# BloodAxe/segmentation-networks-benchmark

Measured on AMD Instinct MI355X. Metric: images/sec/GPU (fwd+bwd) ZF_UNET 224x224 bs=32; 1/2/4/8-GPU scaling, higher is better.
Workload: dtype bf16; 1 GPU; ZF_UNET 224x224 bf16 bs=32/GPU, bce_dice, SGD lr 1e-3, Dropout2d 0.2, train step torch_train.py:180-190 (configs[1]); global_batch=32, parallelism=dp1

## Files before the change

segmentation-networks-benchmark_amd/csrc/common.h:

```cpp
#pragma once
#include <hip/hip_runtime.h>
#include <hip/hip_ext.h>
#include <limits.h>
#include <stdint.h>
#include <stdio.h>
#include <string.h>

#include "../../include/segnb_hip.h"

typedef __attribute__((ext_vector_type(8))) __bf16 bf16x8_t;
typedef __attribute__((ext_vector_type(16))) float f32x16_t;

struct bf16_t {
    unsigned short bits;
};

void segnb_set_error(const char* fmt, ...);

#define SEGNB_CHECK_ARG_AS(who, cond, msg)                           \
    do {                                                             \
        if (!(cond)) {                                               \
            segnb_set_error("%s: bad argument: %s", who, msg);       \
            return SEGNB_E_BADARG;                                   \
        }                                                            \
// ... 35 lines not shown
inline T segnb_plan_keep(T v) {
    static_assert(!(std::is_pointer<T>::value && std::is_class<typename std::remove_pointer<T>::type>::value),
                  "segnb_plan_keep: add an overload that copies this struct into the plan");
    return v;
}
inline const segnb_conv_geom* segnb_plan_keep(const segnb_conv_geom* g) {
    return g ? (const segnb_conv_geom*)segnb_plan_dup(g, sizeof(*g)) : g;
}
inline const segnb_loss_spec* segnb_plan_keep(const segnb_loss_spec* g) {
    return g ? (const segnb_loss_spec*)segnb_plan_dup(g, sizeof(*g)) : g;
}
inline const segnb_bn_reduce_epilogue* segnb_plan_keep(const segnb_bn_reduce_epilogue* g) {
    return g ? (const segnb_bn_reduce_epilogue*)segnb_plan_dup(g, sizeof(*g)) : g;
}
inline const segnb_bn_apply_epilogue* segnb_plan_keep(const segnb_bn_apply_epilogue* g) {
    return g ? (const segnb_bn_apply_epilogue*)segnb_plan_dup(g, sizeof(*g)) : g;
}
inline const segnb_upcat_src* segnb_plan_keep(const segnb_upcat_src* g) {
    return g ? (const segnb_upcat_src*)segnb_plan_dup(g, sizeof(*g)) : g;
}
inline const segnb_operand_tf* segnb_plan_keep(const segnb_operand_tf* g) {
    return g ? (const segnb_operand_tf*)segnb_plan_dup(g, sizeof(*g)) : g;
}
inline const segnb_wgrad_target* segnb_plan_keep(const segnb_wgrad_target* g) {
    return g ? (const segnb_wgrad_target*)segnb_plan_dup(g, sizeof(*g)) : g;
}
inline const segnb_act_epilogue* segnb_plan_keep(const segnb_act_epilogue* g) {
    return g ? (const segnb_act_epilogue*)segnb_plan_dup(g, sizeof(*g)) : g;
}
template <class... P, class... A>
inline void segnb_plan_record_call(const char* name, int (*fn)(P...), A... args) {
    static_assert(sizeof...(P) == sizeof...(A), "argument count");
    std::tuple<P...> kept(segnb_plan_keep((P)args)...);
    segnb_plan_push([fn, kept]() { return std::apply(fn, kept); }, name);
}
extern int g_segnb_census_on;
void segnb_census(const char* name);
#define SEGNB_PLAN_RECORD(fn, ...)                                                           \
    SegnbPlanScope plan_scope__;                                                             \
    if (plan_scope__.top && g_segnb_census_on) segnb_census(#fn);                            \
    if (plan_scope__.top && segnb_plan_recording()) segnb_plan_record_call(#fn, fn, __VA_ARGS__)
void segnb_plan_refuse(const char* why);
#define SEGNB_PLAN_REFUSE(why)                                         \
    SegnbPlanScope plan_scope__;                                       \
    if (plan_scope__.top && g_segnb_census_on) segnb_census(__func__); \
    if (plan_scope__.top && segnb_plan_recording()) segnb_plan_refuse(why)

int segnb_num_cus();
bool segnb_fprop_general_forced();
int segnb_knob_fprop_dma();
int segnb_knob_fprop_dma_cfg();
int segnb_knob_fprop_dma_dbg();
int segnb_knob_fprop_dma_epi();
int segnb_knob_fprop_nostats();
int segnb_knob_rw_store_waves();
int segnb_knob_bnreduce_fused();
int segnb_knob_fprop_deepk();
int segnb_knob_fprop_thin();
enum segnb_try_outcome {
    SEGNB_TRY_DECLINED = 0,
    SEGNB_TRY_LAUNCHED,
    SEGNB_TRY_DELIVERED,
};
constexpr int SEGNB_LAUNCH_DECLINED = INT_MIN;
inline int segnb_try_launched(segnb_try_outcome* did, int rc) {
    if (rc == SEGNB_LAUNCH_DECLINED) {
        *did = SEGNB_TRY_DECLINED;
        return 0;
    }
    if (rc == 0) *did = SEGNB_TRY_LAUNCHED;
    return rc;
}
#define SEGNB_HOST_INLINE static inline __attribute__((always_inline))
template <class... K>
int segnb_opt_in_lds(const char* who, int bytes, K... kernels) {
    hipError_t e = hipSuccess;
    (void)(... && ((e = hipFuncSetAttribute(reinterpret_cast<const void*>(kernels), hipFuncAttributeMaxDynamicSharedMemorySize,
                                            bytes)) == hipSuccess));
    if (e != hipSuccess) segnb_set_error("%s hipFuncSetAttribute(%d bytes): %s", who, bytes, hipGetErrorString(e));
    return (int)e;
}
SEGNB_HOST_INLINE long long segnb_nhwc_bytes(long long npix, int ld, int C, int esz) { return ((npix - 1) * ld + C) * esz; }
SEGNB_HOST_INLINE bool segnb_fits_desc(long long bytes, unsigned* out = nullptr) {
    if (out != nullptr) *out = (unsigned)bytes;
    return bytes < (1ll << 31);
}
inline void segnb_kernel_took(segnb_try_outcome did, const char** served, const char* name) {
    if (did != SEGNB_TRY_DECLINED && *served == nullptr) *served = name;
}
template <class Args>
__attribute__((always_inline)) inline bool take_bn_reduce(Args& a, const segnb_conv_geom* g, const segnb_bn_reduce_epilogue* bn) {
    const long long yb = segnb_nhwc_bytes((long long)g->N * g->Ho * g->Wo, bn->ld_y, g->Co, 2);
    if (!segnb_fits_desc(yb)) return false;
    a.bn_y = (const bf16_t*)bn->y;
    a.bn_y_bytes = (unsigned)yb;
    a.bn_ld = bn->ld_y;
    a.bn_coef = bn->coef;
    a.bn_sums = bn->sums;
    a.bn_act = bn->act;
    a.bn_slope = bn->slope;
    return true;
}
template <class Args>
__attribute__((always_inline)) inline void take_act_epilogue(Args& a, const segnb_act_epilogue* ep) {
    a.ep_act = ep != nullptr ? ep->act : -1;
    a.ep_coef = ep != nullptr ? ep->coef : nullptr;
// ... 221 lines not shown
```

segmentation-networks-benchmark_amd/csrc/fprop_dma.hip:

```cpp
#include "common.h"

#include "fprop_dma.h"

#include <mutex>
#include <vector>

#ifndef SEGNB_EXP
#define SEGNB_EXP 0
#endif

namespace {

__device__ unsigned long long g_stamps[3 * 256 * 4];
#define FD_STAMP(role, step, k)                                                                      \
    do {                                                                                            \
        if (DBG && ((a.dbg & 32) || ((a.dbg & 64) && (role) == 0 && (k) == 0)) && blockIdx.x == 0 && lane == 0 &&  \
            (step) < 256)                                                                            \
            g_stamps[((role) * 256 + (step)) * 4 + (k)] = __builtin_amdgcn_s_memtime();             \
    } while (0)

template <int BN_, int R_, int WT_, int CW_M_, bool TALL_ = false, bool MF16_ = true, int NTAP_ = 9, int UP_ = 0>
struct WsCfg {
    static constexpr bool UPD_ = UP_ == 1;
    static constexpr bool UPF = UP_ == 2;
    static_assert(UP_ == 0 || (NTAP_ == 4 && !TALL_ && MF16_), "up-sampled segment forms: 2 x 2 window, 16x16x32 form");
    static constexpr int BN = BN_, R = R_, WT = WT_;
    static constexpr int NTAP = NTAP_, KW = NTAP_ == 9 ? 3 : 2, KH = KW;
    static constexpr bool UPD = UPD_;
    static constexpr int UP = UP_;
    static constexpr int NPL = UPD_ ? 4 : 1;
    static_assert(NTAP_ == 9 || NTAP_ == 4, "3 x 3 or 2 x 2 tap window");
    static_assert(!UPD_ || (NTAP_ == 4 && !TALL_ && MF16_), "plane gather: 2 x 2 window, 16x16x32 form");
    static constexpr bool TALL = TALL_;
    static constexpr bool MF16 = MF16_;
    static constexpr int BM = TALL_ ? 256 : (R_ * WT_ + 16 * CW_M_ - 1) / (16 * CW_M_) * (16 * CW_M_);
    static constexpr int TM16 = BM / CW_M_ / 16, TN16 = BN_ / (4 / CW_M_) / 16;
    static constexpr int NB = 4;
    static constexpr int NT = 512, NCW = 4, NLW = 4;
    static_assert(R * WT <= BM, "tile pixels");
    static constexpr int NRD = TM16 + TN16, NMF = TM16 * TN16;
    static constexpr int rd_before(int q) { return (q * NRD + NMF - 1) / NMF; }
    static constexpr int WAVES_M = CW_M_, WAVES_N = NCW / CW_M_;
    static constexpr int WM = BM / WAVES_M, WN = BN / WAVES_N;
    static constexpr int TM = WM / 32, TN = WN / 32;
    static constexpr int XR = R + KH - 1, XC = WT + 2, NPIX = XR * XC;
    static constexpr int APIECES = (NPIX + 7) / 8;
    static constexpr int A_BYTES = APIECES * 1024;
    static constexpr int NBW = 2, NAW = 2;
    static constexpr int APW = (APIECES + NAW - 1) / NAW;
    static constexpr int A_STEPS = NTAP - 2;
    static constexpr int APS = (APW + A_STEPS - 1) / A_STEPS;
    static constexpr int BPIECES = BN / 8;
    static constexpr int B_STAGE = BN * 128;
    static constexpr int BPW = BPIECES / NBW;
    static constexpr int OUT_ROW = BN * 2 + 16;
    static constexpr int OC = BN / 8;
    static constexpr int MT = NCW * 64;
    static constexpr int RPT = BM / (MT / OC);
    static constexpr int OFF_B = 2 * A_BYTES;
    static constexpr int OFF_STG = OFF_B + NB * B_STAGE;
    static constexpr int OFF_DUMMY = OFF_STG + BM * OUT_ROW;
    static constexpr int OFF_PIX = OFF_DUMMY + 1024;
    static constexpr int OFF_BIAS = OFF_PIX + 4 * BM * 4;
    static constexpr int OFF_SCALE = OFF_BIAS + BN * 4;
    static constexpr int OFF_TICKET = OFF_SCALE + BN * 4;
    static constexpr int SMEM = OFF_TICKET + 16;
    static constexpr int RED_BYTES = MT * 16 * 8;
    static_assert(WM % (MF16_ ? 16 : 32) == 0 && WN % (MF16_ ? 16 : 32) == 0 && WAVES_M * WAVES_N == NCW, "wave tiling");
    static_assert(BPIECES % NBW == 0 && NBW + NAW == NLW, "fetch wave roles");
    static_assert(MT % OC == 0 && MT >= 2 * BN && RPT <= 8 && BM <= MT && BM % (MT / OC) == 0, "store pass / statistics threads");
    static constexpr bool MASK_OK = MF16_ && !TALL_ && BM == 256 && CW_M_ == 4 && SMEM + 2048 <= 160 * 1024;
    static_assert(RED_BYTES <= OFF_STG, "statistics reduction scratch");
    static_assert(SMEM <= 160 * 1024, "LDS");
    static_assert(TM + TN <= 6, "fragment wait statement");
};

template <class C_>
struct WsEpi : C_ {
    static constexpr bool EPI = true;
};
template <class C, class = void>
struct ws_epi_of : std::false_type {};
template <class C>
struct ws_epi_of<C, std::enable_if_t<C::EPI>> : std::true_type {};

template <class C, bool DBG, bool EP = false, bool STATS = true, bool SPLITK = false, bool MASK = false>
__global__ __launch_bounds__(512) void conv_fprop_ws_kernel(const FdArgs a) {
    static_assert(!SPLITK || (!EP && !DBG && C::UP == 0 && C::NTAP == 9), "split K: plain 3 x 3 forward / data gradient");
    static_assert(!MASK || (STATS && !EP && !DBG && !SPLITK && C::MF16 && C::UP == 0 && C::NTAP == 9 && !C::TALL && C::BM == 256 &&
                            C::BN == 64 && C::WAVES_M == 4 && C::SMEM + 2048 <= 160 * 1024),
                  "activation mask: plain 3 x 3 data gradient, 16x16x32 form, 256 x 64 tiles, 2 KB of mask bytes behind the LDS layout");
    constexpr int BN = C::BN, R = C::R, WT = C::WT, BM = C::BM, TM = C::TM, TN = C::TN, XC = C::XC;
    constexpr int NT = C::NT, NB = C::NB, APW = C::APW, APS = C::APS, BPW = C::BPW, OC = C::OC, NLW = C::NLW;
    constexpr int OUT_ROW = C::OUT_ROW, NF = TM + TN;
    constexpr int NTAP = C::NTAP, KW = C::KW;
    constexpr int SM = NTAP & 3;
    constexpr bool EPI = ws_epi_of<C>::value;
    static_assert(!EPI || (C::MF16 && !SPLITK && !EP && C::UP == 0 && C::NTAP == 9), "store rows in the MFMA gaps: 16x16x32 form, 3 x 3 window, whole-K tiles");

    extern __shared__ __attribute__((aligned(1024))) unsigned char smem[];
    int* sPix = reinterpret_cast<int*>(smem + C::OFF_PIX);
    float* sBias = reinterpret_cast<float*>(smem + C::OFF_BIAS);
    const unsigned lds0 = (unsigned)(size_t)smem;

    const int tid = threadIdx.x, lane = tid & 63, wave = __builtin_amdgcn_readfirstlane(tid >> 6);
    const int r = lane & 31, h = lane >> 5;
    const bool loader = wave >= C::NCW;
    const int lw = wave - C::NCW;
    const int wm = (wave & 3) / C::WAVES_N, wn = (wave & 3) % C::WAVES_N;

    int L_ = xcd_remap(blockIdx.x, gridDim.x);
    int ks_ = 0, nt_, gq_;
    if (C::TALL && a.ntmajor) {
        gq_ = L_ % a.GM;
        L_ /= a.GM;
        if constexpr (SPLITK) {
            ks_ = L_ % a.KS;
            L_ /= a.KS;
        }
        nt_ = L_;
    } else {
        if constexpr (SPLITK) {
            ks_ = L_ % a.KS;
            L_ /= a.KS;
        }
        nt_ = L_ % a.NTL;
        gq_ = L_ / a.NTL;
    }
    const int ks = ks_;
    const int c_off = SPLITK ? ks * a.NCH : 0;
    const int nt = nt_, gq = gq_;
    int n_base_ = nt * BN, w_row0_ = nt * BN, py_ = 0, px_ = 0;
    if constexpr (C::UPF) {
        const int ph = nt / a.NTLR, ct = nt - ph * a.NTLR;
        n_base_ = ct * BN;
        w_row0_ = ph * a.CoW + ct * BN;
        py_ = ph >> 1;
        px_ = ph & 1;
    }
    const int n_base = n_base_, w_row0 = w_row0_, py = py_, px = px_;

    const i32x4_t rs_x = make_rsrc4(a.x, a.x_bytes);
    const i32x4_t rs_w = make_rsrc4(a.w, a.w_bytes);
    const i32x4_t rs_u = make_rsrc4(a.u != nullptr ? a.u : a.x, a.u != nullptr ? a.u_bytes : a.x_bytes);

    float* sScale = reinterpret_cast<float*>(smem + C::OFF_SCALE);
    for (int c = tid; c < BN; c += NT) {
        const int co = n_base + c;
        const float bv = (a.bias != nullptr && co < a.bias_n) ? a.bias[co] : 0.f;
        float sc = 1.f, sh = bv;
        if constexpr (EP) {
// ... 213 lines not shown
                    }
                }
                auto go = [&](auto pl_c) {
                    constexpr int PL = decltype(pl_c)::value;
        #pragma unroll
                    for (int pa = 0; pa < APW; ++pa) {
                        if (pa >= p0 && pa < p1) {
                            const int piece = (lw & 1) + C::NAW * pa;
                            const unsigned dst = piece < C::APIECES ? lds0 + buf * C::A_BYTES + piece * 1024 : lds0 + C::OFF_DUMMY;
                            dma16(dst, a_voff[PL][pa], rs_x, soff);
                        }
                    }
                };
                if constexpr (C::UPD) {
                    if (pl == 0) go(std::integral_constant<int, 0>{});
                    else if (pl == 1) go(std::integral_constant<int, 1>{});
                    else if (pl == 2) go(std::integral_constant<int, 2>{});
                    else go(std::integral_constant<int, 3>{});
                } else {
                    go(std::integral_constant<int, 0>{});
                }
            };
            u32x4_t mreg[MASK ? 16 : 1];
            const __amdgpu_buffer_rsrc_t rs_y = make_rsrc(MASK ? a.bn_y : a.x, MASK ? a.bn_y_bytes : 0);
            auto mask_request = [&](int table) {
                const int t128 = (lw & 1) * 64 + lane;
                const int ch = n_base + (t128 & 7) * 8;
#pragma unroll
                for (int k = 0; k < 16; ++k) {
                    const int opix = sPix[table * BM + (t128 >> 3) + 16 * k];
                    const unsigned voff = (opix >= 0 && ch < a.Co) ? (unsigned)opix * (unsigned)a.bn_ld * 2u + (unsigned)ch * 2u : OOB;
                    mreg[k] = __builtin_amdgcn_raw_buffer_load_b128(rs_y, (int)voff, 0, 0);
                }
            };
            auto mask_publish = [&]() {
                const int t128 = (lw & 1) * 64 + lane;
                unsigned char* const dst = smem + C::SMEM + (t128 >> 3) * 8 + (t128 & 7);
#pragma unroll
                for (int k = 0; k < 16; ++k) {
                    const u32x4_t v = mreg[k];
                    unsigned b = 0u;
                    b |= __uint_as_float(v.x << 16) > 0.f ? 1u : 0u;
                    b |= __uint_as_float(v.x & 0xffff0000u) > 0.f ? 2u : 0u;
                    b |= __uint_as_float(v.y << 16) > 0.f ? 4u : 0u;
                    b |= __uint_as_float(v.y & 0xffff0000u) > 0.f ? 8u : 0u;
                    b |= __uint_as_float(v.z << 16) > 0.f ? 16u : 0u;
                    b |= __uint_as_float(v.z & 0xffff0000u) > 0.f ? 32u : 0u;
                    b |= __uint_as_float(v.w << 16) > 0.f ? 64u : 0u;
                    b |= __uint_as_float(v.w & 0xffff0000u) > 0.f ? 128u : 0u;
                    dst[16 * k * 8] = (unsigned char)b;
                }
                asm volatile("s_waitcnt lgkmcnt(0)" ::: "memory");
            };
            set_fetch_tile(it, 0);
            fetch_a(0, APW, 0, 0);
            if (a.NCH == 1) set_fetch_tile(it + a.GM, 1);
            asm volatile("s_waitcnt vmcnt(0)" ::: "memory");
            lds_barrier();
            int tile_no = 0;
            for (; it < a.IT; it += a.GM, ++tile_no) {
                for (int c = 0; c < a.NCH; ++c, ++cg) {
                    const bool last = c + 1 == a.NCH;
                    const int cn = last ? 0 : c + 1;
                    const bool next_last = last ? a.NCH == 1 : c + 2 == a.NCH;
                    const int setup_it = last ? it + 2 * a.GM : it + a.GM;
                    const int setup_tab = (tile_no + (last ? 2 : 1)) & 3;
                    const int abuf = cg & 1;
                    static_for<NTAP>([&](auto t_c) {
                        constexpr int t = decltype(t_c)::value;
                        if (lw == C::NBW) FD_STAMP(2, cg * 9 + t, 0);
                        if constexpr (t < C::A_STEPS)
                            if (!(SEGNB_EXP & 2) && !(DBG && (a.dbg & 2))) fetch_a(t * APS, (t + 1) * APS, cn, abuf ^ 1);
                        if constexpr (MASK) {
                            if constexpr (t == 0)
                                if (c == 0) mask_request(tile_no & 3);
                            if constexpr (t == NTAP - 1)
                                if (last) mask_publish();
                        }
                        if constexpr (t == NTAP - 2)
                            if (next_last) set_fetch_tile(setup_it, setup_tab);
                        if (lw == C::NBW) FD_STAMP(2, cg * 9 + t, 1);
                        if constexpr (t == NTAP - 2) {
                            asm volatile("s_waitcnt vmcnt(0)" ::: "memory");
                        }
                        if (lw == C::NBW) FD_STAMP(2, cg * 9 + t, 2);
                        if (!(SEGNB_EXP & 64) || t % 3 == 2) raw_barrier();
                        if (lw == C::NBW) FD_STAMP(2, cg * 9 + t, 3);
                    });
                }
            }
        }
        asm volatile("s_waitcnt vmcnt(0)" ::: "memory");
        if constexpr (SPLITK) {
            raw_barrier();
            raw_barrier();
        }
        raw_barrier();
        raw_barrier();
        raw_barrier();
    } else {
        constexpr bool MF16 = C::MF16;
        int tile_no_out = 0;
        bool pending_out = false;
        constexpr int TM16 = C::TM16, TN16 = C::TN16;
        int b_rd[MF16 ? 1 : TN];
        int a_rd[MF16 ? 1 : 9][MF16 ? 1 : TM];
        static_assert(!MF16 || XC % 2 == 0, "16x16x32 form: the swizzle key must be the halo column");
        int b_rd16[MF16 ? 2 : 1][MF16 ? TN16 : 1];
        int a_rd16[MF16 ? KW : 1][MF16 ? TM16 : 1][MF16 ? 2 : 1];
        if constexpr (MF16) {
            const int r16 = lane & 15, g4 = lane >> 4;
    #pragma unroll
            for (int j = 0; j < TN16; ++j) {
                const int row = wn * C::WN + 16 * j + r16;
                const int v = C::OFF_B + row * 128 + ((g4 ^ ((row >> 1) & 7)) << 4);
                b_rd16[0][j] = v;
                b_rd16[1][j] = v ^ 64;
            }
    #pragma unroll
            for (int dwi = 0; dwi < KW; ++dwi)
    #pragma unroll
                for (int i = 0; i < TM16; ++i) {
                    const int m_ = wm * C::WM + 16 * i + r16;
                    const int m = (R * WT == BM || m_ < R * WT) ? m_ : 0;
                    const int p = (m / WT) * XC + (m % WT) + a.dw[dwi];
                    const int key = p % XC;
                    int v = (p << 7) + ((g4 ^ ((key >> 1) & 7)) << 4);
                    asm volatile("" : "+v"(v));
                    a_rd16[dwi][i][0] = v;
                    a_rd16[dwi][i][1] = v ^ 64;
                }
        } else {
        #pragma unroll
            for (int j = 0; j < TN; ++j) {
                const int row = wn * C::WN + 32 * j + r;
                b_rd[j] = C::OFF_B + row * 128 + ((row & 12) << 3) + (((h ^ (row >> 1)) & 1) << 4);
            }
        #pragma unroll
            for (int t = 0; t < 9; ++t)
        #pragma unroll
                for (int i = 0; i < TM; ++i) {
                    const int m = wm * C::WM + 32 * i + r;
// ... 618 lines not shown
        if (e == nullptr) {
            ents.push_back(Ent{dev, stream, nullptr, 0, nullptr, 0});
            e = &ents.back();
        }
        if (slab_bytes > e->cap) {
            float* p = nullptr;
            if (hipMalloc(&p, slab_bytes) != hipSuccess) return -1;
            e->slab = p;
            e->cap = slab_bytes;
        }
        if (ntiles > e->ncnt) {
            const int want = ntiles < 1024 ? 1024 : ntiles;
            int* c = nullptr;
            if (hipMalloc(&c, (size_t)want * sizeof(int)) != hipSuccess) return -1;
            if (hipMemsetAsync(c, 0, (size_t)want * sizeof(int), stream) != hipSuccess) return -1;
            e->cnt = c;
            e->ncnt = want;
        }
    }
    *slab = e->slab;
    *cnt = e->cnt;
    return 0;
}

template <class C>
int ksplit_factor(const FdArgs& a, int it_total, int ntl, int nch) {
    if (!C::TALL || !segnb_knob_fprop_ksplit()) return 1;
    if (a.ep_act >= 0 || a.dbg || a.up_out != nullptr) return 1;
    const long long tiles = (long long)it_total * ntl;
    int cus = segnb_knob_conv_cus();
    if (a.stats == nullptr) cus /= 2;
    int ks = 1;
    if (tiles * 2 <= cus && nch % 2 == 0 && nch / 2 >= 2) ks = 2;
    if (tiles * 4 <= cus && nch % 4 == 0 && nch / 4 >= 2) ks = 4;
    const int forced = segnb_knob_fprop_ksplit();
    if (forced > 1 && nch % forced == 0 && nch / forced >= 2 && (forced == 2 || forced == 4)) ks = forced;
    if (tiles * ks * 65536ll >= (1ll << 31)) return 1;
    return ks;
}

template <class C>
constexpr bool ws_has_epi() {
    return C::MF16 && !C::TALL && C::BN == 64 && C::NTAP == 9 && ((C::R == 14 && C::WT == 14) || (C::R == 16 && C::WT == 16));
}
bool ws_epi_selected(bool by_default) {
    const int k = segnb_knob_fprop_dma_epi();
    const bool on = k < 0 ? by_default : k != 0;
    if (on && g_segnb_census_on) segnb_census("epi:1");
    return on;
}
constexpr bool WS_EPI_DEFAULT = true;

template <class C>
int launch_ws(FdArgs& a, hipStream_t stream) {
    if (a.bn_y != nullptr && !C::MASK_OK) return SEGNB_LAUNCH_DECLINED;
    static const int attr_rc = [] {
        int rc = segnb_opt_in_lds("fprop_ws", C::SMEM, conv_fprop_ws_kernel<C, false>, conv_fprop_ws_kernel<C, true>,
                                  conv_fprop_ws_kernel<C, false, true, false>, conv_fprop_ws_kernel<C, false, false, false>);
        if constexpr (C::MASK_OK) {
            if (rc == 0) rc = segnb_opt_in_lds("fprop_ws", C::SMEM + 2048, conv_fprop_ws_kernel<C, false, false, true, false, true>);
        }
        if constexpr (C::TALL) {
            if (rc == 0)
                rc = segnb_opt_in_lds("fprop_ws", C::SMEM, conv_fprop_ws_kernel<C, false, false, true, true>,
                                      conv_fprop_ws_kernel<C, false, false, false, true>);
        }
        if constexpr (ws_has_epi<C>()) {
            using CE = WsEpi<C>;
            if (rc == 0)
                rc = segnb_opt_in_lds("fprop_ws", C::SMEM, conv_fprop_ws_kernel<CE, false>, conv_fprop_ws_kernel<CE, true>,
                                      conv_fprop_ws_kernel<CE, false, false, false>);
            if constexpr (C::MASK_OK) {
                if (rc == 0) rc = segnb_opt_in_lds("fprop_ws", C::SMEM + 2048, conv_fprop_ws_kernel<CE, false, false, true, false, true>);
            }
        }
        return rc;
    }();
    if (attr_rc) return attr_rc;
    a.HB = (a.H + C::R - 1) / C::R;
    a.WB = (a.W + C::WT - 1) / C::WT;
    a.IT = a.N * a.HB * a.WB;
    if (C::TALL) {
        if (a.W > C::WT || a.Hi != a.H || a.Wi != a.W) return SEGNB_LAUNCH_DECLINED;
        a.IT = (a.N * (a.H + 1) + C::R - 1) / C::R;
    }
    a.NTL = (a.Co + C::BN - 1) / C::BN;
    a.NCH = a.Ci / 64;
    a.KS = 1;
    a.ntmajor = C::TALL ? 1 : 0;
    if constexpr (C::TALL) {
        const int ks = ksplit_factor<C>(a, a.IT, a.NTL, a.NCH);
        if (ks > 1 && ksplit_workspace(stream, (size_t)a.IT * a.NTL * ks * 65536, a.IT * a.NTL, &a.ks_slab, &a.ks_cnt) == 0) {
            a.KS = ks;
            a.NCH /= ks;
            a.GM = a.IT;
            a.ks_slab_bytes = (unsigned)((size_t)a.IT * a.NTL * ks * 65536);
            const dim3 grid(a.IT * a.NTL * ks);
            if (a.stats != nullptr || !segnb_knob_fprop_nostats())
                hipLaunchKernelGGL((conv_fprop_ws_kernel<C, false, false, true, true>), grid, dim3(C::NT), C::SMEM, stream, a);
            else
                hipLaunchKernelGGL((conv_fprop_ws_kernel<C, false, false, false, true>), grid, dim3(C::NT), C::SMEM, stream, a);
            return 0;
        }
    }
    int gm = segnb_knob_conv_cus() / a.NTL;
    if (gm < 1) gm = 1;
    if (gm > a.IT) gm = a.IT;
    a.GM = gm;
    if constexpr (ws_has_epi<C>()) {
        if (a.ep_act < 0 && ws_epi_selected(WS_EPI_DEFAULT)) {
            using CE = WsEpi<C>;
            const dim3 grid(a.GM * a.NTL), block(C::NT);
            if (a.bn_y != nullptr) {
                if constexpr (C::MASK_OK)
                    hipLaunchKernelGGL((conv_fprop_ws_kernel<CE, false, false, true, false, true>), grid, block, C::SMEM + 2048, stream, a);
                else
                    return SEGNB_LAUNCH_DECLINED;
            } else if (a.stats == nullptr && !a.dbg && segnb_knob_fprop_nostats())
                hipLaunchKernelGGL((conv_fprop_ws_kernel<CE, false, false, false>), grid, block, C::SMEM, stream, a);
            else if (a.dbg)
                hipLaunchKernelGGL((conv_fprop_ws_kernel<CE, true>), grid, block, C::SMEM, stream, a);
            else
                hipLaunchKernelGGL((conv_fprop_ws_kernel<CE, false>), grid, block, C::SMEM, stream, a);
            return 0;
        }
    }
    if (a.bn_y != nullptr) {
        if constexpr (C::MASK_OK) {
            hipLaunchKernelGGL((conv_fprop_ws_kernel<C, false, false, true, false, true>), dim3(a.GM * a.NTL), dim3(C::NT), C::SMEM + 2048,
                               stream, a);
            return 0;
        } else {
            return SEGNB_LAUNCH_DECLINED;
        }
    }
    if (a.ep_act >= 0)
        hipLaunchKernelGGL((conv_fprop_ws_kernel<C, false, true, false>), dim3(a.GM * a.NTL), dim3(C::NT), C::SMEM, stream, a);
    else if (a.stats == nullptr && !a.dbg && segnb_knob_fprop_nostats())
        hipLaunchKernelGGL((conv_fprop_ws_kernel<C, false, false, false>), dim3(a.GM * a.NTL), dim3(C::NT), C::SMEM, stream, a);
    else if (a.dbg)
        hipLaunchKernelGGL((conv_fprop_ws_kernel<C, true>), dim3(a.GM * a.NTL), dim3(C::NT), C::SMEM, stream, a);
    else
        hipLaunchKernelGGL((conv_fprop_ws_kernel<C, false>), dim3(a.GM * a.NTL), dim3(C::NT), C::SMEM, stream, a);
    return 0;
}

using WsCfg14 = WsCfg<64, 14, 14, 2, false, true>;

bool ws14_serves(const FdArgs& a) {
    return a.H % 14 == 0 && a.W % 14 == 0 && a.W <= 56 && a.Co > 32 && a.bn_y == nullptr && a.ep_act < 0 && !a.dbg &&
           a.up_out == nullptr && segnb_knob_fprop_mf16();
}

int launch_ws14(FdArgs& a, hipStream_t stream) {
    using C = WsCfg14;
    using CE = WsEpi<C>;
    static const int attr_rc = segnb_opt_in_lds("fprop_ws", C::SMEM, conv_fprop_ws_kernel<C, false>, conv_fprop_ws_kernel<C, false, false, false>,
                                                conv_fprop_ws_kernel<CE, false>, conv_fprop_ws_kernel<CE, false, false, false>);
    if (attr_rc) return attr_rc;
    a.HB = a.H / C::R;
    a.WB = a.W / C::WT;
    a.IT = a.N * a.HB * a.WB;
    a.NTL = (a.Co + C::BN - 1) / C::BN;
    a.NCH = a.Ci / 64;
    a.KS = 1;
    a.ntmajor = 0;
    int gm = segnb_knob_conv_cus() / a.NTL;
    if (gm < 1) gm = 1;
    if (gm > a.IT) gm = a.IT;
    a.GM = gm;
    if (g_segnb_census_on) segnb_census("tile:ws14");
    if (ws_epi_selected(WS_EPI_DEFAULT)) {
        if (a.stats == nullptr && segnb_knob_fprop_nostats())
            hipLaunchKernelGGL((conv_fprop_ws_kernel<CE, false, false, false>), dim3(a.GM * a.NTL), dim3(C::NT), C::SMEM, stream, a);
        else
            hipLaunchKernelGGL((conv_fprop_ws_kernel<CE, false>), dim3(a.GM * a.NTL), dim3(C::NT), C::SMEM, stream, a);
        return 0;
    }
    if (a.stats == nullptr && segnb_knob_fprop_nostats())
        hipLaunchKernelGGL((conv_fprop_ws_kernel<C, false, false, false>), dim3(a.GM * a.NTL), dim3(C::NT), C::SMEM, stream, a);
    else
        hipLaunchKernelGGL((conv_fprop_ws_kernel<C, false>), dim3(a.GM * a.NTL), dim3(C::NT), C::SMEM, stream, a);
    return 0;
}

template <class C>
int launch_ws_upd(FdArgs& a, hipStream_t stream) {
    static const int attr_rc = segnb_opt_in_lds("fprop_ws", C::SMEM, conv_fprop_ws_kernel<C, false, false, false>);
    if (attr_rc) return attr_rc;
    a.HB = (a.H + C::R - 1) / C::R;
    a.WB = (a.W + C::WT - 1) / C::WT;
    a.IT = a.N * a.HB * a.WB;
    a.NTL = (a.Co + C::BN - 1) / C::BN;
    a.P32 = a.Ci == 32;
    a.NCHP = a.P32 ? 1 : a.Ci / 64;
    a.NCH = a.P32 ? 2 : 4 * a.NCHP;
    a.RPS = a.NCH * C::NTAP - 1 < C::RPT ? 2 : 1;
    if ((a.NCH * C::NTAP - 1) * a.RPS < C::RPT) return SEGNB_LAUNCH_DECLINED;
    int gm = segnb_knob_conv_cus() / a.NTL;
    if (gm < 1) gm = 1;
    if (gm > a.IT) gm = a.IT;
    a.GM = gm;
    hipLaunchKernelGGL((conv_fprop_ws_kernel<C, false, false, false>), dim3(a.GM * a.NTL), dim3(C::NT), C::SMEM, stream, a);
    return 0;
}

template <class C>
int launch_ws_upf(FdArgs& a, hipStream_t stream) {
    static const int attr_rc = segnb_opt_in_lds("fprop_ws", C::SMEM, conv_fprop_ws_kernel<C, false, false, true>);
    if (attr_rc) return attr_rc;
    a.HB = (a.H + C::R - 1) / C::R;
    a.WB = (a.W + C::WT - 1) / C::WT;
    a.IT = a.N * a.HB * a.WB;
    a.NTLR = (a.Co + C::BN - 1) / C::BN;
    a.NTL = 4 * a.NTLR;
    a.NCH = a.Ci / 64;
    a.NCHP = a.NCH;
    a.P32 = 0;
    a.RPS = a.NCH * C::NTAP - 1 < C::RPT ? 2 : 1;
    if ((a.NCH * C::NTAP - 1) * a.RPS < C::RPT) return SEGNB_LAUNCH_DECLINED;
    int gm = segnb_knob_conv_cus() / a.NTL;
    if (gm < 1) gm = 1;
    if (gm > a.IT) gm = a.IT;
    a.GM = gm;
    hipLaunchKernelGGL((conv_fprop_ws_kernel<C, false, false, true>), dim3(a.GM * a.NTL), dim3(C::NT), C::SMEM, stream, a);
// ... 221 lines not shown
```

segmentation-networks-benchmark_amd/csrc/runtime.hip:

```cpp
#include <stdarg.h>
#include <stdlib.h>

#include "common.h"

static thread_local char g_err[512] = "";

void segnb_set_error(const char* fmt, ...) {
    va_list ap;
    va_start(ap, fmt);
    vsnprintf(g_err, sizeof(g_err), fmt, ap);
    va_end(ap);
}

int segnb_num_cus() {
    static int cus = 0;
    if (cus > 0) return cus;
    int dev = 0;
    hipDeviceProp_t prop;
    if (hipGetDevice(&dev) != hipSuccess || hipGetDeviceProperties(&prop, dev) != hipSuccess) return 256;
    cus = prop.multiProcessorCount > 0 ? prop.multiProcessorCount : 256;
    return cus;
}

extern "C" const char* segnb_last_error(void) { return g_err; }
// ... 260 lines not shown
        const char* e = getenv("SEGNB_FPROP_MF16");
        g_fprop_mf16 = (e != nullptr && e[0] == '0') ? 0 : 1;
    }
    return g_fprop_mf16;
}
static int g_fprop_upd = -2;
int segnb_knob_fprop_upd() {
    if (g_fprop_upd == -2) {
        const char* e = getenv("SEGNB_FPROP_UPD");
        g_fprop_upd = (e != nullptr && e[0] == '0') ? 0 : 1;
    }
    return g_fprop_upd;
}
static int g_fprop_mask = -2;
int segnb_knob_fprop_mask() {
    if (g_fprop_mask == -2) {
        const char* e = getenv("SEGNB_FPROP_MASK");
        g_fprop_mask = (e != nullptr && e[0] == '0') ? 0 : 1;
    }
    return g_fprop_mask;
}
static int g_fprop_drop = -2;
int segnb_knob_fprop_drop() {
    if (g_fprop_drop == -2) {
        const char* e = getenv("SEGNB_FPROP_DROP");
        g_fprop_drop = (e != nullptr && e[0] == '0') ? 0 : 1;
    }
    return g_fprop_drop;
}
static int g_fprop_nostats = 1;
int segnb_knob_fprop_nostats() { return g_fprop_nostats; }
static int g_rw_store_waves = 4;
int segnb_knob_rw_store_waves() { return g_rw_store_waves; }
static int g_bnreduce_fused = -2;
int segnb_knob_bnreduce_fused() {
    if (g_bnreduce_fused == -2) {
        const char* e = getenv("SEGNB_BNREDUCE_FUSED");
        g_bnreduce_fused = (e != nullptr && e[0] == '0') ? 0 : 1;
    }
    return g_bnreduce_fused;
}
static int g_fprop_ksplit = -2;
int segnb_knob_fprop_ksplit() {
    if (g_fprop_ksplit == -2) {
        const char* e = getenv("SEGNB_FPROP_KSPLIT");
        g_fprop_ksplit = e != nullptr ? atoi(e) : 1;
    }
    return g_fprop_ksplit;
}
static int g_fprop_dma_dbg = 0;
int segnb_knob_fprop_dma_dbg() { return g_fprop_dma_dbg; }
static int g_fprop_dma_epi = -1;
int segnb_knob_fprop_dma_epi() { return g_fprop_dma_epi; }
extern "C" int segnb_wg_cu_share(int pct) {
    SEGNB_PLAN_RECORD(segnb_wg_cu_share, pct);
    g_wg_cu_pct = pct < 0 ? 0 : (pct > 100 ? 100 : pct);
    return 0;
}

static thread_local segnb_wgrad_target g_wg_target;
static thread_local bool g_wg_target_armed = false;
extern "C" int segnb_wgrad_target_arm(const segnb_wgrad_target* t) {
    SEGNB_PLAN_RECORD(segnb_wgrad_target_arm, t);
    SEGNB_CHECK_ARG(t != nullptr && t->gw != nullptr, "NULL target");
    SEGNB_CHECK_ARG(t->ntaps >= 1 && t->ntaps <= SEGNB_MAX_TAPS && t->Ci > 0 && t->Co > 0 && t->s_in >= t->ntaps && t->ci_off >= 0 &&
                        t->s_out >= (long long)(t->ci_off + t->Ci) * t->s_in, "bad target layout");
    for (int i = 0; i < t->ntaps; ++i) SEGNB_CHECK_ARG(t->kpos[i] >= 0 && t->kpos[i] < t->s_in, "bad kernel position");
    g_wg_target = *t;
    g_wg_target_armed = true;
    return 0;
}
const segnb_wgrad_target* segnb_take_wgrad_target() {
    if (!g_wg_target_armed) return nullptr;
    g_wg_target_armed = false;
    return &g_wg_target;
}

extern "C" int segnb_tune(const char* key, int value) {
    SEGNB_PLAN_REFUSE("segnb_tune inside a recorded plan");
    SEGNB_CHECK_ARG(key != nullptr, "NULL key");
    if (strcmp(key, "fprop_dma") == 0) {
        g_fprop_dma = value ? 1 : 0;
        return 0;
    }
    if (strcmp(key, "fprop_dma_cfg") == 0) {
        g_fprop_dma_cfg = value < 0 ? -1 : value;
        return 0;
    }
    if (strcmp(key, "fprop_roll") == 0) {
        g_fprop_roll = value < 0 ? 0 : value;
        return 0;
    }
    if (strcmp(key, "pack_blocks") == 0) {
        g_pack_blocks = value < 0 ? 0 : value;
        return 0;
    }
    if (strcmp(key, "wgrad_roll") == 0) {
        g_wgrad_roll = value ? 1 : 0;
        return 0;
    }
    if (strcmp(key, "wgrad_c8roll") == 0) {
        g_wgrad_c8roll = value ? 1 : 0;
        return 0;
    }
    if (strcmp(key, "fprop_rw") == 0) {
        g_fprop_rw = value ? 1 : 0;
// ... 6 lines not shown
    if (strcmp(key, "plan_profile") == 0) {
        if (value == 2) plan_profile_dump();
        else g_plan_profile = value;
        return 0;
    }
    if (strcmp(key, "wg_cu_pct") == 0) {
        g_wg_cu_pct = value < 0 ? 0 : (value > 100 ? 100 : value);
        return 0;
    }
    if (strcmp(key, "fprop_drop") == 0) {
        g_fprop_drop = value ? 1 : 0;
        return 0;
    }
    if (strcmp(key, "fprop_mask") == 0) {
        g_fprop_mask = value ? 1 : 0;
        return 0;
    }
    if (strcmp(key, "fprop_nostats") == 0) {
        g_fprop_nostats = value ? 1 : 0;
        return 0;
    }
    if (strcmp(key, "rw_store_waves") == 0) {
        g_rw_store_waves = value == 2 ? 2 : (value == 8 ? 8 : 4);
        return 0;
    }
    if (strcmp(key, "bnreduce_fused") == 0) {
        g_bnreduce_fused = value ? 1 : 0;
        return 0;
    }
    if (strcmp(key, "fprop_deepk") == 0) {
        g_fprop_deepk = value ? 1 : 0;
        return 0;
    }
    if (strcmp(key, "fprop_thin") == 0) {
        g_fprop_thin = value ? 1 : 0;
        return 0;
    }
    if (strcmp(key, "fprop_mf16") == 0) {
        g_fprop_mf16 = value ? 1 : 0;
        return 0;
    }
    if (strcmp(key, "call_census") == 0) {
        g_segnb_census_on = value ? 1 : 0;
        return 0;
    }
    if (strcmp(key, "fprop_ksplit") == 0) {
        g_fprop_ksplit = value < 0 ? 0 : value;
        return 0;
    }
    if (strcmp(key, "fprop_dma_epi") == 0) {
        g_fprop_dma_epi = value < 0 ? -1 : (value ? 1 : 0);
        return 0;
    }
    if (strcmp(key, "fprop_dma_dbg") == 0) {
        g_fprop_dma_dbg = value;
        return 0;
    }
    segnb_set_error("segnb_tune: unknown key '%s'", key);
    return SEGNB_E_BADARG;
}

extern "C" int segnb_debug_stamps(unsigned long long* host_dst) {
    SEGNB_CHECK_ARG(host_dst != nullptr, "NULL destination");
    return segnb_fprop_dma_read_stamps(host_dst);
}
```

Baseline: 7062 images/s.

## Precompute next-tile fetch offsets with edge bitmasks and double-buffered offset sets

Adds a switched loader path to the warp-specialized forward convolution. Tile-boundary validity is precomputed once per lane as bitmasks for the first and last row and column tiles. The next tile's address offsets and pixel table are built incrementally inside the current tile's last chunk and held in a second offset set that alternates parity. This takes per-tile address and bounds recomputation off the loader waves' critical path between tiles. The cost is more registers, more kernel instantiations, and a separability precondition that falls back to the old path when it is not met.

```diff
diff --git a/segmentation-networks-benchmark_amd/csrc/common.h b/segmentation-networks-benchmark_amd/csrc/common.h
--- a/segmentation-networks-benchmark_amd/csrc/common.h
+++ b/segmentation-networks-benchmark_amd/csrc/common.h
@@ -111,6 +111,7 @@
 int segnb_knob_fprop_dma_cfg();
 int segnb_knob_fprop_dma_dbg();
 int segnb_knob_fprop_dma_epi();
+int segnb_knob_fprop_dma_switch();
 int segnb_knob_fprop_nostats();
 int segnb_knob_rw_store_waves();
 int segnb_knob_bnreduce_fused();
diff --git a/segmentation-networks-benchmark_amd/csrc/fprop_dma.hip b/segmentation-networks-benchmark_amd/csrc/fprop_dma.hip
--- a/segmentation-networks-benchmark_amd/csrc/fprop_dma.hip
+++ b/segmentation-networks-benchmark_amd/csrc/fprop_dma.hip
@@ -1,6 +1,7 @@
 #include "common.h"
 
 #include "fprop_dma.h"
+#include "ws_switch.h"
 
 #include <mutex>
 #include <vector>
@@ -83,6 +84,14 @@
 struct ws_epi_of : std::false_type {};
 template <class C>
 struct ws_epi_of<C, std::enable_if_t<C::EPI>> : std::true_type {};
+template <class C_>
+struct WsSwitch : C_ {
+    static constexpr bool SWITCH = true;
+};
+template <class C, class = void>
+struct ws_switch_of : std::false_type {};
+template <class C>
+struct ws_switch_of<C, std::enable_if_t<C::SWITCH>> : std::true_type {};
 
 template <class C, bool DBG, bool EP = false, bool STATS = true, bool SPLITK = false, bool MASK = false>
 __global__ __launch_bounds__(512) void conv_fprop_ws_kernel(const FdArgs a) {
@@ -97,6 +106,9 @@
     constexpr int SM = NTAP & 3;
     constexpr bool EPI = ws_epi_of<C>::value;
     static_assert(!EPI || (C::MF16 && !SPLITK && !EP && C::UP == 0 && C::NTAP == 9), "store rows in the MFMA gaps: 16x16x32 form, 3 x 3 window, whole-K tiles");
+    constexpr bool SW = ws_switch_of<C>::value;
+    static_assert(!SW || (EPI && !C::TALL && C::APW <= 32 && C::R % 2 == 0 && C::WT % 2 == 0 && C::XC % 2 == 0),
+                  "second offset set: the WsEpi forms; one bit per piece; even tiles (virtual concat: tile origin / 2 is exact)");
 
     extern __shared__ __attribute__((aligned(1024))) unsigned char smem[];
     int* sPix = reinterpret_cast<int*>(smem + C::OFF_PIX);
@@ -416,6 +428,140 @@
                 }
                 asm volatile("s_waitcnt lgkmcnt(0)" ::: "memory");
             };
+            if constexpr (SW) {
+            unsigned u_rel[APW], a_vo[2][APW], a_uo[2][APW];
+            const bool vc = !MASK && vcat;
+            const WsEdgeBits eb = ws_edge_bits(lw & 1, C::NAW, APW, lane, XC, C::NPIX, R, WT, a.HB, a.WB, a.dhmin, a.dwmin, a.Hi, a.Wi);
+        #pragma unroll
+            for (int pa = 0; pa < APW; ++pa) {
+                const int pix = ws_piece_pixel((lw & 1) + C::NAW * pa, lane);
+                const int xr = pix / XC, xc = pix - xr * XC;
+                u_rel[pa] = vc ? (unsigned)(((xr + a.dhmin) >> 1) * a.Wu + ((xc + a.dwmin) >> 1)) * (unsigned)a.ld_u * 2u +
+                                       (unsigned)(((lane & 7) ^ ((xc >> 1) & 7)) * 16)
+                                 : 0u;
+            }
+            constexpr int NTB = (BM + C::NAW * 64 - 1) / (C::NAW * 64);
+            const int t128 = (lw & 1) * 64 + lane;
+            int t_ro[NTB], t_co[NTB];
+        #pragma unroll
+            for (int j = 0; j < NTB; ++j) {
+                const int rr = t128 + j * C::NAW * 64;
+                const bool in_tile = rr < BM && rr < R * WT;
+                t_ro[j] = in_tile ? rr / WT : 0x7fffffff;
+                t_co[j] = rr % WT;
+            }
+            const WsTilePos step = ws_tile_pos(a.GM, a.HB, a.WB);
+            WsTilePos pos = ws_tile_pos(it, a.HB, a.WB);
+            int sit = it;
+            unsigned nx_base = 0u, nx_ubase = 0u, nx_bad = ~0u;
+            int nx_obase = 0, nx_hrem = 0, nx_wrem = 0;
+            auto setup_begin = [&]() {
+                const bool live = sit < a.IT;
+                const int h0 = pos.hb * R + a.dhmin, w0 = pos.wb * WT + a.dwmin;
+                nx_base = (unsigned)(((pos.n * a.Hi + h0) * a.Wi + w0) * a.ld_x * 2);
+                nx_ubase = vc ? (unsigned)((pos.n * a.Hu + pos.hb * (R / 2)) * a.Wu + pos.wb * (WT / 2)) * (unsigned)a.ld_u * 2u : 0u;
+                nx_bad = ws_tile_bad(eb, pos, a.HB, a.WB, live);
+                nx_obase = (pos.n * a.H + pos.hb * R) * a.W + pos.wb * WT;
+                nx_hrem = live ? a.H - pos.hb * R : 0;
+                nx_wrem = a.W - pos.wb * WT;
+            };
+            auto setup_entries = [&](auto set_c, int p0, int p1) {
+                constexpr int S = decltype(set_c)::value;
+        #pragma unroll
+                for (int pa = 0; pa < APW; ++pa) {
+                    if (pa >= p0 && pa < p1) {
+                        const bool ok = ((nx_bad >> pa) & 1u) == 0u;
+                        a_vo[S][pa] = ok ? nx_base + a_rel[pa] : OOB;
+                        if (vc) a_uo[S][pa] = ok ? nx_ubase + u_rel[pa] : OOB;
+                    }
+                }
+            };
+            auto setup_end = [&](int table) {
+        #pragma unroll
+                for (int j = 0; j < NTB; ++j) {
+                    const int rr = t128 + j * C::NAW * 64;
+                    if (rr < BM) sPix[table * BM + rr] = (t_ro[j] < nx_hrem && t_co[j] < nx_wrem) ? nx_obase + (int)((unsigned)t_ro[j] * (unsigned)a.W) + t_co[j] : -1;
+                }
+                ws_tile_advance(pos, step, a.HB, a.WB);
+                sit += a.GM;
+            };
+            auto fetch_sw = [&](auto set_c, int p0, int p1, int c, int buf) {
+                constexpr int S = decltype(set_c)::value;
+                const bool from_u = vc && c < a.NCHU;
+                const unsigned soff = vc && !from_u ? (unsigned)(c - a.NCHU) * 128u : (unsigned)c * 128u;
+                auto go = [&](const unsigned (&off)[APW], const i32x4_t& rs) {
+        #pragma unroll
+                    for (int pa = 0; pa < APW; ++pa) {
+                        if (pa >= p0 && pa < p1) {
+                            const int piece = (lw & 1) + C::NAW * pa;
+                            const unsigned dst = piece < C::APIECES ? lds0 + buf * C::A_BYTES + piece * 1024 : lds0 + C::OFF_DUMMY;
+                            dma16(dst, off[pa], rs, soff);
+                        }
+                    }
+                };
+                if (from_u)
+                    go(a_uo[S], rs_u);
+                else
+                    go(a_vo[S], rs_x);
+            };
+            constexpr std::integral_constant<int, 0> S0{};
+            setup_begin();
+            setup_entries(S0, 0, APW);
+            setup_end(0);
+            fetch_sw(S0, 0, APW, 0, 0);
+            if (a.NCH == 1) {
+                setup_begin();
+                setup_entries(S0, 0, APW);
+                setup_end(1);
+            }
+            asm volatile("s_waitcnt vmcnt(0)" ::: "memory");
+            lds_barrier();
+            int tile_no = 0, par = 0;
+            for (; it < a.IT; it += a.GM, ++tile_no) {
+                for (int c = 0; c < a.NCH; ++c, ++cg) {
+                    const bool last = c + 1 == a.NCH;
+                    const int cn = last ? 0 : c + 1;
+                    const bool next_last = last ? a.NCH == 1 : c + 2 == a.NCH;
+                    const int setup_tab = (tile_no + (last ? 2 : 1)) & 3;
+                    const int abuf = cg & 1;
+                    auto chunk = [&](auto par_c) {
+                        constexpr int P = decltype(par_c)::value;
+                        static_for<NTAP>([&](auto t_c) {
+                            constexpr int t = decltype(t_c)::value;
+                            if (lw == C::NBW) FD_STAMP(2, cg * 9 + t, 0);
+                            if constexpr (t < C::A_STEPS) {
+                                if (!(SEGNB_EXP & 2) && !(DBG && (a.dbg & 2))) fetch_sw(par_c, t * APS, (t + 1) * APS, cn, abuf ^ 1);
+                                if (next_last) {
+                                    if constexpr (t == 0) setup_begin();
+                                    if constexpr (SEGNB_EXP & 512) __builtin_amdgcn_s_setprio(2);
+                                    setup_entries(std::integral_constant<int, P ^ 1>{}, t * APS, (t + 1) * APS);
+                                    if constexpr (t == C::A_STEPS - 1) setup_end(setup_tab);
+                                    if constexpr (SEGNB_EXP & 512) __builtin_amdgcn_s_setprio(0);
+                                }
+                            }
+                            if constexpr (MASK) {
+                                if constexpr (t == 0)
+                                    if (c == 0) mask_request(tile_no & 3);
+                                if constexpr (t == NTAP - 1)
+                                    if (last) mask_publish();
+                            }
+                            if (lw == C::NBW) FD_STAMP(2, cg * 9 + t, 1);
+                            if constexpr (t == NTAP - 2) {
+                                asm volatile("s_waitcnt vmcnt(0)" ::: "memory");
+                            }
+                            if (lw == C::NBW) FD_STAMP(2, cg * 9 + t, 2);
+                            raw_barrier();
+                            if (lw == C::NBW) FD_STAMP(2, cg * 9 + t, 3);
+                        });
+                    };
+                    if (par)
+                        chunk(std::integral_constant<int, 1>{});
+                    else
+                        chunk(S0);
+                    if (next_last) par ^= 1;
+                }
+            }
+            } else {
             set_fetch_tile(it, 0);
             fetch_a(0, APW, 0, 0);
             if (a.NCH == 1) set_fetch_tile(it + a.GM, 1);
@@ -452,6 +598,7 @@
                         if (lw == C::NBW) FD_STAMP(2, cg * 9 + t, 3);
                     });
                 }
+            }
             }
         }
         asm volatile("s_waitcnt vmcnt(0)" ::: "memory");
@@ -1176,6 +1323,16 @@
 constexpr bool WS_EPI_DEFAULT = true;
 
 template <class C>
+bool ws_switch_selected(const FdArgs& a, bool by_default) {
+    const int k = segnb_knob_fprop_dma_switch();
+    const bool on = (k < 0 ? by_default : k != 0) && ws_edges_separable(a.HB, C::R, C::XR, a.dhmin, a.Hi) &&
+                    ws_edges_separable(a.WB, C::WT, C::XC, a.dwmin, a.Wi);
+    if (on && g_segnb_census_on) segnb_census("switch:1");
+    return on;
+}
+constexpr bool WS_SWITCH_DEFAULT_16 = true, WS_SWITCH_DEFAULT_14 = true;
+
+template <class C>
 int launch_ws(FdArgs& a, hipStream_t stream) {
     if (a.bn_y != nullptr && !C::MASK_OK) return SEGNB_LAUNCH_DECLINED;
     static const int attr_rc = [] {
@@ -1196,6 +1353,13 @@
                                       conv_fprop_ws_kernel<CE, false, false, false>);
             if constexpr (C::MASK_OK) {
                 if (rc == 0) rc = segnb_opt_in_lds("fprop_ws", C::SMEM + 2048, conv_fprop_ws_kernel<CE, false, false, true, false, true>);
+            }
+            using CS = WsSwitch<CE>;
+            if (rc == 0)
+                rc = segnb_opt_in_lds("fprop_ws", C::SMEM, conv_fprop_ws_kernel<CS, false>, conv_fprop_ws_kernel<CS, true>,
+                                      conv_fprop_ws_kernel<CS, false, false, false>);
+            if constexpr (C::MASK_OK) {
+                if (rc == 0) rc = segnb_opt_in_lds("fprop_ws", C::SMEM + 2048, conv_fprop_ws_kernel<CS, false, false, true, false, true>);
             }
         }
         return rc;
@@ -1233,20 +1397,25 @@
     a.GM = gm;
     if constexpr (ws_has_epi<C>()) {
         if (a.ep_act < 0 && ws_epi_selected(WS_EPI_DEFAULT)) {
-            using CE = WsEpi<C>;
             const dim3 grid(a.GM * a.NTL), block(C::NT);
-            if (a.bn_y != nullptr) {
-                if constexpr (C::MASK_OK)
-                    hipLaunchKernelGGL((conv_fprop_ws_kernel<CE, false, false, true, false, true>), grid, block, C::SMEM + 2048, stream, a);
+            auto launch = [&](auto cfg) {
+                using CE = decltype(cfg);
+                if (a.bn_y != nullptr) {
+                    if constexpr (C::MASK_OK)
+                        hipLaunchKernelGGL((conv_fprop_ws_kernel<CE, false, false, true, false, true>), grid, block, C::SMEM + 2048, stream, a);
+                    else
+                        return SEGNB_LAUNCH_DECLINED;
+                } else if (a.stats == nullptr && !a.dbg && segnb_knob_fprop_nostats())
+                    hipLaunchKernelGGL((conv_fprop_ws_kernel<CE, false, false, false>), grid, block, C::SMEM, stream, a);
+                else if (a.dbg)
+                    hipLaunchKernelGGL((conv_fprop_ws_kernel<CE, true>), grid, block, C::SMEM, stream, a);
                 else
-                    return SEGNB_LAUNCH_DECLINED;
-            } else if (a.stats == nullptr && !a.dbg && segnb_knob_fprop_nostats())
-                hipLaunchKernelGGL((conv_fprop_ws_kernel<CE, false, false, false>), grid, block, C::SMEM, stream, a);
-            else if (a.dbg)
-                hipLaunchKernelGGL((conv_fprop_ws_kernel<CE, true>), grid, block, C::SMEM, stream, a);
-            else
-                hipLaunchKernelGGL((conv_fprop_ws_kernel<CE, false>), grid, block, C::SMEM, stream, a);
-            return 0;
+                    hipLaunchKernelGGL((conv_fprop_ws_kernel<CE, false>), grid, block, C::SMEM, stream, a);
+                return 0;
+            };
+            if ((a.bn_y == nullptr || C::MASK_OK) && ws_switch_selected<C>(a, C::R == 14 ? WS_SWITCH_DEFAULT_14 : WS_SWITCH_DEFAULT_16))
+                return launch(WsSwitch<WsEpi<C>>{});
+            return launch(WsEpi<C>{});
         }
     }
     if (a.bn_y != nullptr) {
@@ -1279,8 +1448,10 @@
 int launch_ws14(FdArgs& a, hipStream_t stream) {
     using C = WsCfg14;
     using CE = WsEpi<C>;
+    using CS = WsSwitch<CE>;
     static const int attr_rc = segnb_opt_in_lds("fprop_ws", C::SMEM, conv_fprop_ws_kernel<C, false>, conv_fprop_ws_kernel<C, false, false, false>,
-                                                conv_fprop_ws_kernel<CE, false>, conv_fprop_ws_kernel<CE, false, false, false>);
+                                                conv_fprop_ws_kernel<CE, false>, conv_fprop_ws_kernel<CE, false, false, false>,
+                                                conv_fprop_ws_kernel<CS, false>, conv_fprop_ws_kernel<CS, false, false, false>);
     if (attr_rc) return attr_rc;
     a.HB = a.H / C::R;
     a.WB = a.W / C::WT;
@@ -1295,6 +1466,13 @@
     a.GM = gm;
     if (g_segnb_census_on) segnb_census("tile:ws14");
     if (ws_epi_selected(WS_EPI_DEFAULT)) {
+        if (ws_switch_selected<C>(a, WS_SWITCH_DEFAULT_14)) {
+            if (a.stats == nullptr && segnb_knob_fprop_nostats())
+                hipLaunchKernelGGL((conv_fprop_ws_kernel<CS, false, false, false>), dim3(a.GM * a.NTL), dim3(C::NT), C::SMEM, stream, a);
+            else
+                hipLaunchKernelGGL((conv_fprop_ws_kernel<CS, false>), dim3(a.GM * a.NTL), dim3(C::NT), C::SMEM, stream, a);
+            return 0;
+        }
         if (a.stats == nullptr && segnb_knob_fprop_nostats())
             hipLaunchKernelGGL((conv_fprop_ws_kernel<CE, false, false, false>), dim3(a.GM * a.NTL), dim3(C::NT), C::SMEM, stream, a);
         else
diff --git a/segmentation-networks-benchmark_amd/csrc/runtime.hip b/segmentation-networks-benchmark_amd/csrc/runtime.hip
--- a/segmentation-networks-benchmark_amd/csrc/runtime.hip
+++ b/segmentation-networks-benchmark_amd/csrc/runtime.hip
@@ -336,6 +336,8 @@
 int segnb_knob_fprop_dma_dbg() { return g_fprop_dma_dbg; }
 static int g_fprop_dma_epi = -1;
 int segnb_knob_fprop_dma_epi() { return g_fprop_dma_epi; }
+static int g_fprop_dma_switch = -1;
+int segnb_knob_fprop_dma_switch() { return g_fprop_dma_switch; }
 extern "C" int segnb_wg_cu_share(int pct) {
     SEGNB_PLAN_RECORD(segnb_wg_cu_share, pct);
     g_wg_cu_pct = pct < 0 ? 0 : (pct > 100 ? 100 : pct);
@@ -448,6 +450,10 @@
         g_fprop_dma_epi = value < 0 ? -1 : (value ? 1 : 0);
         return 0;
     }
+    if (strcmp(key, "fprop_dma_switch") == 0) {
+        g_fprop_dma_switch = value < 0 ? -1 : (value ? 1 : 0);
+        return 0;
+    }
     if (strcmp(key, "fprop_dma_dbg") == 0) {
         g_fprop_dma_dbg = value;
         return 0;
diff --git a/segmentation-networks-benchmark_amd/csrc/ws_switch.h b/segmentation-networks-benchmark_amd/csrc/ws_switch.h
--- /dev/null
+++ b/segmentation-networks-benchmark_amd/csrc/ws_switch.h
@@ -0,0 +1,68 @@
+#pragma once
+
+#if defined(__HIPCC__) || defined(__CUDACC__)
+#define WS_HD __host__ __device__ inline
+#else
+#define WS_HD inline
+#endif
+
+struct WsTilePos {
+    int n, hb, wb;
+};
+
+WS_HD WsTilePos ws_tile_pos(int it, int HB, int WB) {
+    WsTilePos p;
+    p.n = it / (HB * WB);
+    const int rem = it - p.n * (HB * WB);
+    p.hb = rem / WB;
+    p.wb = rem - p.hb * WB;
+    return p;
+}
+
+WS_HD void ws_tile_advance(WsTilePos& p, const WsTilePos& step, int HB, int WB) {
+    p.wb += step.wb;
+    const int cw = p.wb >= WB ? 1 : 0;
+    p.wb -= cw ? WB : 0;
+    p.hb += step.hb + cw;
+    const int ch = p.hb >= HB ? 1 : 0;
+    p.hb -= ch ? HB : 0;
+    p.n += step.n + ch;
+}
+
+WS_HD bool ws_axis_valid(int t, int x, int T, int dmin, int lim) { return (unsigned)(t * T + dmin + x) < (unsigned)lim; }
+
+WS_HD bool ws_edges_separable(int nt, int T, int XT, int dmin, int lim) {
+    if (nt <= 1) return true;
+    return T + dmin >= 0 && (nt - 2) * T + dmin + XT - 1 < lim;
+}
+
+struct WsEdgeBits {
+    unsigned row_first, row_last, col_first, col_last, pad;
+};
+
+WS_HD int ws_piece_pixel(int piece, int lane) { return piece * 8 + (lane >> 3); }
+
+WS_HD WsEdgeBits ws_edge_bits(int first_piece, int piece_step, int npieces, int lane, int XC, int NPIX, int R, int WT, int HB, int WB,
+                              int dhmin, int dwmin, int Hi, int Wi) {
+    WsEdgeBits b = {0u, 0u, 0u, 0u, 0u};
+    for (int pa = 0; pa < npieces; ++pa) {
+        const int pix = ws_piece_pixel(first_piece + piece_step * pa, lane);
+        const int xr = pix / XC, xc = pix - xr * XC;
+        const unsigned bit = 1u << pa;
+        if (pix >= NPIX) b.pad |= bit;
+        if (!ws_axis_valid(0, xr, R, dhmin, Hi)) b.row_first |= bit;
+        if (!ws_axis_valid(HB - 1, xr, R, dhmin, Hi)) b.row_last |= bit;
+        if (!ws_axis_valid(0, xc, WT, dwmin, Wi)) b.col_first |= bit;
+        if (!ws_axis_valid(WB - 1, xc, WT, dwmin, Wi)) b.col_last |= bit;
+    }
+    return b;
+}
+
+WS_HD unsigned ws_tile_bad(const WsEdgeBits& b, const WsTilePos& p, int HB, int WB, bool live) {
+    unsigned bad = b.pad;
+    bad |= p.hb == 0 ? b.row_first : 0u;
+    bad |= p.hb == HB - 1 ? b.row_last : 0u;
+    bad |= p.wb == 0 ? b.col_first : 0u;
+    bad |= p.wb == WB - 1 ? b.col_last : 0u;
+    return live ? bad : ~0u;
+}
```

Result: no change. 7107 images/s (median of 6 runs) (+0.6%).
